# Fancomi2017/InstanceFusion

Hardware: AMD Instinct MI355X
Metric: frames/s + ms/frame (ICP|fuse|instance) at 640x480, 5M surfels, 1/2/4/8 GPU (higher is better)
Workload: dtype f32; 1 GPU; 5000000-surfel map, 640x480 synthetic RGBD stream, 3-level ICP+RGB + surfel fuse + canned-mask instance votes with superpixel refinement; surfels_live=4734799, surfel_slots=4734799, map_order=random, parallelism=replicas x1, loop_frames=90

## Files before the change

include/ifx_c_api.h:

```cpp
#ifndef IFX_C_API_H_
#define IFX_C_API_H_

#include <stdint.h>

#ifdef __cplusplus
extern "C" {
#endif

#define IFX_NUM_INSTANCES 96
#define IFX_VOTE_FLOATS 48

enum {
    IFX_OK = 0,
    IFX_E_INVALID = -1,
    IFX_E_HIP = -2,
    IFX_E_CAPACITY = -3,
    IFX_E_STATE = -4
};

typedef struct ifx_config {
    int32_t width, height;
    float fx, fy, cx, cy;
    int32_t time_delta;
    float confidence;
// ... 46 lines not shown
int ifx_owner_comm_ranks(ifx_t* h);
int ifx_owner_exchange(ifx_t* h, int phase, void** ptrs, int64_t* bytes, int32_t* ops, int max_n);
int ifx_owner_predict_phase(ifx_t* h, int step);
int ifx_owner_of(const float* xyz, int n, int n_ranks, int32_t* out);
int ifx_owner_segmentation_begin(ifx_t* h, const uint8_t* rgb, const uint16_t* depth, const uint8_t* masks, const int32_t* class_ids, int nm, int frame, int flags);
int ifx_owner_segmentation_resume(ifx_t* h);
int ifx_owner_ids_begin(ifx_t* h);
int ifx_owner_ids_resume(ifx_t* h);
int ifx_owner_knn_export(ifx_t* h, void** d_points, void** d_labels, int* n);
int ifx_owner_knn_vote(ifx_t* h, const void* d_all_points, const void* d_all_labels, int n_all, int own_offset);
int ifx_map_seq(ifx_t* h, uint32_t* out, int max_n);
int ifx_map_bounding_boxes(ifx_t* h, int bbox_type, float ratio, float* boxes96x6, float* ground_normal3, float* gc_matrix16, float* inst_matrix96x16,
                           int32_t* ground_votes648);
int ifx_instance_point_cloud(ifx_t* h, int bbox_type, int32_t* counts96, int inst, float* out10, int max_records);
int ifx_view_list_stats(ifx_t* h, int32_t* out4);
int ifx_sync(ifx_t* h);
int ifx_get_pose(ifx_t* h, float* out_pose16);
int ifx_tick(ifx_t* h);
int ifx_trajectory(ifx_t* h, float* out_poses16, int max_frames);
int ifx_tracker_diag(ifx_t* h, float* diag8);
int ifx_tracker_fallbacks(ifx_t* h);
int ifx_tracker_range_exceeded(ifx_t* h);
int ifx_tracker_meet_giveups(ifx_t* h);

int ifx_set_loop_closure(ifx_t* h, int enable, int count_thresh, float err_thresh, float cov_thresh);
int ifx_loop_closure_diag(ifx_t* h, float* out24);
typedef int (*ifx_loop_closure_cb)(ifx_t* h, const float* lc24, void* user);
int ifx_set_loop_closure_callback(ifx_t* h, ifx_loop_closure_cb cb, void* user);
int ifx_sample_graph_model(ifx_t* h, float* out_xyzt, int max_n);
int ifx_loop_closure_constraints(ifx_t* h, float* src3, float* dst3, int32_t* times, int max_n);
int ifx_set_deformation(ifx_t* h, const float* graph16, int n_nodes, int is_fern);
int ifx_adopt_estimated_pose(ifx_t* h);

typedef int (*ifx_fern_cb)(ifx_t* h, void* user);
int ifx_set_fern_callback(ifx_t* h, ifx_fern_cb cb, void* user);
int ifx_adopt_pose(ifx_t* h, const float* pose16);
int ifx_fern_frame(ifx_t* h, uint8_t* img_rgb, float* verts4, float* norms4, uint8_t* inst_rgb);
int ifx_fern_frame_async(ifx_t* h);
int ifx_fern_frame_fetch(ifx_t* h, uint8_t* img_rgb, float* verts4, float* norms4, uint8_t* inst_rgb);
int ifx_track_maps(ifx_t* h, const float* model_v4, const float* model_n4, const uint8_t* model_rgba, const float* cur_v4, const float* cur_n4,
                   const uint8_t* cur_rgba, float* pose16, float* diag8);

typedef struct ifx_soa_view {
    int32_t count;
    int32_t capacity;
    float* d_pos_conf;
// ... 202 lines not shown
```

instancefusion_amd/__init__.py:

```python
from __future__ import annotations

import ctypes as C
import os

import numpy as np

_HERE = os.path.dirname(os.path.abspath(__file__))
LIB_PATH = os.environ.get("IFX_LIB") or os.path.join(_HERE, "libifx.so")
HEADER_PATH = os.path.join(os.path.dirname(_HERE), "include", "ifx_c_api.h")

NUM_INSTANCES = 96
VOTE_FLOATS = 48


class IfxError(RuntimeError):
    pass


class IfxConfig(C.Structure):
    _fields_ = [
        ("width", C.c_int32), ("height", C.c_int32),
        ("fx", C.c_float), ("fy", C.c_float), ("cx", C.c_float), ("cy", C.c_float),
        ("time_delta", C.c_int32), ("confidence", C.c_float), ("depth_cut", C.c_float),
        ("max_depth_processed", C.c_float), ("icp_weight", C.c_float),
# ... 89 lines not shown
    "ifx_owner_process_frame": (C.c_int, [_P, _P, _P, C.c_int64, _P]),
    "ifx_owner_predict": (C.c_int, [_P]),
    "ifx_owner_process_segmentation": (C.c_int, [_P, _P, _P, _P, _P, C.c_int, C.c_int, C.c_int]),
    "ifx_owner_knn_vote_colour": (C.c_int, [_P]),
    "ifx_owner_exchange_stats": (C.c_int, [_P, _P, C.c_int]),
    "ifx_owner_comm_ranks": (C.c_int, [_P]),
    "ifx_map_seq": (C.c_int, [_P, _P, C.c_int]),
    "ifx_prefetch_frame_device": (C.c_int, [_P, _P, _P]),
    "ifx_hint_next_frame_device": (C.c_int, [_P, _P, _P]),
    "ifx_hint_next_frame": (C.c_int, [_P, _P, _P]),
    "ifx_lookahead_stats": (C.c_int, [_P, _P, C.c_int]),
    "ifx_view_list_stats": (C.c_int, [_P, _P]),
    "ifx_map_bounding_boxes": (C.c_int, [_P, C.c_int, C.c_float, _P, _P, _P, _P, _P]),
    "ifx_instance_point_cloud": (C.c_int, [_P, C.c_int, _P, C.c_int, _P, C.c_int]),
    "ifx_sync": (C.c_int, [_P]),
    "ifx_get_pose": (C.c_int, [_P, _P]),
    "ifx_tick": (C.c_int, [_P]),
    "ifx_trajectory": (C.c_int, [_P, _P, C.c_int]),
    "ifx_tracker_diag": (C.c_int, [_P, _P]),
    "ifx_tracker_fallbacks": (C.c_int, [_P]),
    "ifx_build_pyramids": (C.c_int, [_P, _P, _P, _P, _P, _P, _P, C.POINTER(Pyramids)]),
    "ifx_tracker_range_exceeded": (C.c_int, [_P]),
    "ifx_tracker_meet_giveups": (C.c_int, [_P]),
    "ifx_hot_records_stale": (C.c_int, [_P]),
    "ifx_set_loop_closure": (C.c_int, [_P, C.c_int, C.c_int, C.c_float, C.c_float]),
    "ifx_loop_closure_diag": (C.c_int, [_P, _P]),
    "ifx_set_loop_closure_callback": (C.c_int, [_P, _P, _P]),
    "ifx_sample_graph_model": (C.c_int, [_P, _P, C.c_int]),
    "ifx_loop_closure_constraints": (C.c_int, [_P, _P, _P, _P, C.c_int]),
    "ifx_set_deformation": (C.c_int, [_P, _P, C.c_int, C.c_int]),
    "ifx_adopt_estimated_pose": (C.c_int, [_P]),
    "ifx_set_fern_callback": (C.c_int, [_P, _P, _P]),
    "ifx_adopt_pose": (C.c_int, [_P, _P]),
    "ifx_fern_frame": (C.c_int, [_P, _P, _P, _P, _P]),
    "ifx_fern_frame_async": (C.c_int, [_P]),
    "ifx_fern_frame_fetch": (C.c_int, [_P, _P, _P, _P, _P]),
    "ifx_track_maps": (C.c_int, [_P, _P, _P, _P, _P, _P, _P, _P, _P]),
    "ifx_map_view": (C.c_int, [_P, C.POINTER(SoaView)]),
    "ifx_map_count": (C.c_int, [_P]),
    "ifx_map_slots": (C.c_int, [_P]),
    "ifx_map_download": (C.c_int, [_P, C.c_int] + [_P] * 6),
    "ifx_map_upload": (C.c_int, [_P, C.c_int] + [_P] * 6),
    "ifx_set_pose": (C.c_int, [_P, _P, C.c_int]),
    "ifx_compact": (C.c_int, [_P]),
    "ifx_set_option": (C.c_int, [_P, C.c_char_p, C.c_int]),
    "ifx_ids_after": (_P, [_P]),
# ... 238 lines not shown
    @property
    def tick(self):
        return self.L.ifx_tick(self.handle)

    def trajectory(self, max_frames=1 << 16):
        out = np.zeros((max_frames, 16), np.float32)
        n = self._chk(self.L.ifx_trajectory(self.handle, _ptr(out), max_frames), "ifx_trajectory")
        return out[:n].reshape(n, 4, 4).copy()

    def tracker_diag(self):
        out = np.zeros(8, np.float32)
        self._chk(self.L.ifx_tracker_diag(self.handle, _ptr(out)), "ifx_tracker_diag")
        return out

    def tracker_fallbacks(self):
        return self._chk(self.L.ifx_tracker_fallbacks(self.handle), "ifx_tracker_fallbacks")

    def tracker_range_exceeded(self):
        return self._chk(self.L.ifx_tracker_range_exceeded(self.handle), "ifx_tracker_range_exceeded")

    def tracker_meet_giveups(self):
        return self._chk(self.L.ifx_tracker_meet_giveups(self.handle), "ifx_tracker_meet_giveups")

    def set_loop_closure(self, enable=True, count_thresh=35000, err_thresh=5e-5, cov_thresh=1e-5):
        self._chk(self.L.ifx_set_loop_closure(self.handle, int(enable), int(count_thresh), err_thresh, cov_thresh), "ifx_set_loop_closure")

    def loop_closure_diag(self):
        out = np.zeros(24, np.float32)
        self._chk(self.L.ifx_loop_closure_diag(self.handle, _ptr(out)), "ifx_loop_closure_diag")
        return dict(ran=bool(out[0]), inactive_pixels=int(out[1]), icp_error=float(out[2]), icp_count=float(out[3]), cov_ok=bool(out[4]),
                    accepted=bool(out[5]), est_pose=out[6:22].reshape(4, 4).copy(), cov_max=float(out[22]), candidates=int(out[23]))

    def set_loop_closure_callback(self, fn):
        if fn is None:
            self._lc_cb = None
            self._chk(self.L.ifx_set_loop_closure_callback(self.handle, None, None), "ifx_set_loop_closure_callback")
            return

        def tramp(_h, lc, _user):
            try:
                fn(self, np.ctypeslib.as_array(lc, shape=(24,)).copy())
                return 0
            except Exception:
                import traceback

                traceback.print_exc()
# ... 508 lines not shown
```

instancefusion_amd/csrc/ifx_api.hip:

```cpp
#include <climits>
#include "ifx_ctx.h"
#include <string.h>
#include <stdio.h>
#include <algorithm>

int ifx_tracker_external_pose(ifx* h, const float* d_pose16, float weight_mult);
int ifx_tracker_set_weight(ifx* h, float weight_mult);
int ifx_compact_enqueue(ifx* h, int refresh_ids);

void hs_invalidate_view(ifx* h);
static std::string g_err;
extern "C" const char* ifx_global_error(void) { return g_err.c_str(); }
extern "C" const char* ifx_last_error(ifx_t* h) { return h ? h->err.c_str() : g_err.c_str(); }

hipEvent_t ifx_event_get(ifx* h)
{
    if (!h->event_pool.empty()) { hipEvent_t e = h->event_pool.back(); h->event_pool.pop_back(); return e; }
    hipEvent_t e;
    hipEventCreate(&e);
    return e;
}
void ifx_ktime_begin(ifx* h, const char* name, hipEvent_t* a)
{
    (void)name;
// ... 341 lines not shown
    }
    else if (s == "seg_snapshots") { if (value < 1 || value > 8) { h->err = "seg_snapshots must be in [1, 8]"; return IFX_E_INVALID; } h->opt_seg_snapshots = value; }
    else if (s == "ff_rounds") h->opt_ff_rounds = value;
    else if (s == "gn_persist_blocks") { if (value < 1) return IFX_E_INVALID; ifx_drop_tracked(h); h->opt_gn_persist_blocks = value; }
    else if (s == "gn_persist") {
        if (value < 0 || value > 7) { h->err = "gn_persist is a mask of pyramid levels (0..7)"; return IFX_E_INVALID; }
        ifx_drop_tracked(h);
        h->opt_gn_persist = value;
    }
    else if (s == "gn_spin_limit" || s == "gn_fault") {
        if (value < 0) return IFX_E_INVALID;
        ifx_drop_tracked(h);
        HIPCHK(h, hipStreamSynchronize(h->stream));
        HIPCHK(h, hipMemcpy((char*)h->d_state + (s == "gn_fault" ? offsetof(DevState, gn_fault) : offsetof(DevState, gn_spin_limit)), &value, sizeof(int), hipMemcpyHostToDevice));
    }
    else if (s == "gn_prologue") { ifx_drop_tracked(h); h->opt_gn_prologue = value ? 1 : 0; }
    else if (s == "rgb_cand") { ifx_drop_tracked(h); h->opt_rgb_cand = value ? 1 : 0; }
    else if (s == "rgb_fuse") {
        if (value < 0 || value > 7) { h->err = "rgb_fuse is a mask of pyramid levels (0..7)"; return IFX_E_INVALID; }
        ifx_drop_tracked(h);
        h->opt_rgb_fuse = value;
    }
    else if (s == "rgb_fuse_poll") { ifx_drop_tracked(h); h->opt_rgb_fuse_poll = value ? 1 : 0; }
    else if (s == "raster_lds") h->opt_raster_lds = value;
    else if (s == "raster_earlyz") h->opt_raster_earlyz = value;
    else if (s == "pyramid" || s == "fast_odom" || s == "so3" || s == "icp_weight_x1000") {
        if (h->hint_rgb || h->slot[h->tick & 1].for_tick == h->tick) { h->err = "tracker options cannot change while a frame is announced ahead"; return IFX_E_STATE; }
        ifx_drop_tracked(h);
        if (s == "pyramid") h->cfg.pyramid = value ? 1 : 0;
        else if (s == "fast_odom") h->cfg.fast_odom = value ? 1 : 0;
        else if (s == "so3") h->cfg.so3 = value ? 1 : 0;
        else { if (value < 0 || value > 100000) { h->err = "icp_weight_x1000 must be in [0, 100000]"; return IFX_E_INVALID; } h->cfg.icp_weight = value / 1000.f; }
    }
    else { h->err = "unknown option " + s; return IFX_E_INVALID; }
    return IFX_OK;
}

__global__ void k_frame_result(DevState* __restrict__ st, FrameResult* __restrict__ out, float* __restrict__ traj_slot)
{
    if (threadIdx.x < 64) frame_result_wave(st, out, traj_slot, 0, (int)threadIdx.x);
}

static int enqueue_frame_side(ifx* h, int s, int tick, const uint8_t* rgb, const uint16_t* depth, int src_kind)
{
    FrameSlot& f = h->slot[s];
    const int bound = h->cur_slot;
// ... 750 lines not shown
    HIPCHK(h, hipStreamSynchronize(h->stream));
    HIPCHK(h, hipStreamSynchronize(h->stream_b));
    if (h->stream_c) HIPCHK(h, hipStreamSynchronize(h->stream_c));
    ktime_flush(h);
    stage_flush(h);
    if (h->h_result->overflow) { h->err = "surfel store capacity exceeded"; return IFX_E_CAPACITY; }
    return IFX_OK;
}
extern "C" int ifx_tracker_fallbacks(ifx_t* h)
{
    if (!h) return IFX_E_INVALID;
    int r = ifx_sync(h);
    return r ? r : h->h_result->gn_timeout;
}

extern "C" int ifx_hot_records_stale(ifx_t* h)
{
    if (!h) return IFX_E_INVALID;
    HIPCHK(h, hipStreamSynchronize(h->stream));
    int v = 0;
    HIPCHK(h, hipMemcpy(&v, &h->d_state->hot_stale, sizeof(int), hipMemcpyDeviceToHost));
    return v;
}
extern "C" int ifx_tracker_meet_giveups(ifx_t* h)
{
    if (!h) return IFX_E_INVALID;
    int r = ifx_sync(h);
    if (r) return r;
    if (h->stream_c) HIPCHK(h, hipStreamSynchronize(h->stream_c));
    if (h->stream_b) HIPCHK(h, hipStreamSynchronize(h->stream_b));
    long long total = 0;
    for (const DevState* d : {(const DevState*)h->d_state, (const DevState*)h->d_cam_trk}) {
        if (!d) continue;
        int v = 0;
        HIPCHK(h, hipMemcpy(&v, (const char*)d + offsetof(DevState, rgb_meet_giveups), sizeof(int), hipMemcpyDeviceToHost));
        total += v;
    }
    return (int)std::min<long long>(total, 0x7FFFFFFF);
}
extern "C" int ifx_tracker_range_exceeded(ifx_t* h)
{
    if (!h) return IFX_E_INVALID;
    int r = ifx_sync(h);
    if (r) return r;
    if (h->stream_c) HIPCHK(h, hipStreamSynchronize(h->stream_c));
    if (h->stream_b) HIPCHK(h, hipStreamSynchronize(h->stream_b));
    std::vector<const DevState*> sts;
    sts.push_back(h->d_state);
    if (h->d_m2m) sts.push_back(h->d_m2m);
    if (h->d_cam_trk) sts.push_back(h->d_cam_trk);
    for (const FrameSlot& f : h->slot) if (f.so3) sts.push_back(f.so3);
    long long total = 0;
    for (const DevState* d : sts) {
        int v = 0;
        HIPCHK(h, hipMemcpy(&v, (const char*)d + offsetof(DevState, range_exceeded), sizeof(int), hipMemcpyDeviceToHost));
        total += v;
    }
    return (int)std::min<long long>(total, 0x7FFFFFFF);
}

static int frame_sync(ifx* h)
{
// ... 388 lines not shown
```

instancefusion_amd/csrc/ifx_ctx.h:

```cpp
#pragma once
#include <hip/hip_runtime.h>
#include <stdint.h>
#include <string>
#include <vector>
#include <map>
#include "../../include/ifx_c_api.h"
#include "ifx_dev.h"

#ifndef IFX_LIST_SEGS
#define IFX_LIST_SEGS 8
#endif

struct DevState {
    float pose[16];
    float pose_inv[16];
    float last_pose[16];
    float weighting;
    int dense_enough;
    int count;
    int n_dead;
    int n_new;
    int overflow;
    unsigned int r_max_bits;
    float Rprev[9], tprev[3], Rprev_inv[9];
// ... 27 lines not shown
    int vl_valid;
    int vl_scan;
    int vl_age;
    int vl_scans;
    unsigned int vl_n[2];
    unsigned int vl_seg_n[2 * IFX_LIST_SEGS], vl_seg_off[2 * IFX_LIST_SEGS];
    long long dbg[8];
    alignas(64) int gn_res[2];
    unsigned int gn_ticket;
    int gn_pad[13];
    double gn_acc[2 * IFX_ACC_REPL * IFX_ACC_STRIDE];
    double gn_acc2[2 * 2 * IFX_ACC_REPL * IFX_ACC_STRIDE];
    alignas(64) int gn_res2[2 * 16];
    alignas(64) unsigned int gn_bar[4 * 32 * 16];
    int gn_timeout;
    int gn_abort;
    int gn_done_seq;
    int gn_spin_limit, gn_fault;
    alignas(64) double gnp_acc[3 * 2 * IFX_ACC_REPL * IFX_ACC_STRIDE];
    alignas(64) int gnp_res[3 * 16];
    alignas(64) unsigned int gnp_meet[3 * 32];
    alignas(64) double gnp_RRt[2][16];
    int rgb_meet_giveups;
};

struct IdMap { const uint32_t* seq; int own_n; };
__device__ __forceinline__ int idmap_slot(const IdMap& m, int count, int id)
{
    if (m.own_n <= 0) return (id > 0 && id < count) ? id : -1;
    if (id == 0) return -1;
    int lo = 0, hi = count - 1;
    while (lo <= hi) {
        const int mid = (lo + hi) >> 1;
        const unsigned int v = m.seq[mid];
        if (v == (unsigned int)id) return mid;
        if (v < (unsigned int)id) lo = mid + 1; else hi = mid - 1;
    }
    return -1;
}

struct FrameResult {
    float pose[16];
    float diag[8];
    int count, n_dead, n_new, overflow;
    int gn_timeout;
    int seg_counts[2];
// ... 213 lines not shown
    int opt_gn_persist_blocks = 128;
    int opt_gn_persist = 0;
    int gn_max_blocks[4] = {0, 0, 0, 0};
    int opt_rgb_blocks = 0;
    int opt_gn_prologue = 1;
    int oseg_state = 0, oseg_nm = 0, oseg_m = 0, oseg_flags = 0, oseg_pending = 0;
    std::vector<uint8_t> oseg_unavail;
    std::vector<int> oseg_cmp, oseg_bbox, oseg_class;
    hipEvent_t oseg_ev = nullptr;
    int32_t* oseg_rec = nullptr;
    size_t oseg_rec_cap = 0, oseg_rec_bytes = 0;
    int oseg_root = -1, oseg_form = 0, oseg_M = 0, oseg_maxn = 0;
    float oseg_thr = 0.f;
    const char* oseg_who = "";
    void* d_kexp = nullptr;
    int gn_begin_folded = 0;
    int labels_stale_all = 1;
    int opt_raster_lds = 0;
    int opt_view_blocks = 0, opt_clean_blocks = 0, opt_index_blocks = 0;
    int icp_resident_blocks = 1024;
    int opt_res_blocks = 0;
    int opt_rgb_cand = 1;
    int opt_rgb_fuse = 7;
    int opt_rgb_fuse_poll = 1;
    int icp_resident_blocks_fuse = 1024;
    int opt_icp_blocks = 0;
    int opt_raster_tiles = -1;
    int map_external = 0;
    int lc_enable = 0, lc_count_thresh = 35000;
    float lc_err_thresh = 5e-5f, lc_cov_thresh = 1e-5f;
    DevState* d_m2m = nullptr;
    Pyr m2m;
    float *old_vertex = nullptr, *old_normal = nullptr;
    uint8_t *old_image = nullptr, *old_inst = nullptr;
    uint16_t* old_time = nullptr;
    float *act_vertex = nullptr, *act_normal = nullptr;
    uint8_t *act_image = nullptr, *act_inst = nullptr;
    uint16_t* act_time = nullptr;
    size_t lc_half = 0;
    int own_tracked_tick = 0;
    float* h_lc = nullptr;
    int lc_event_valid = 0;
    float* d_graph = nullptr;
    int graph_nodes = 0, graph_is_fern = 0;
    uint8_t* d_inst_gt = nullptr;
    int inst_gt_on = 0;
// ... 208 lines not shown
```

instancefusion_amd/csrc/ifx_track.hip:

```cpp
#include "ifx_ctx.h"
#include "ifx_rgb_chunks.h"
#include <math.h>
#include <string.h>


#define BIL_R 6
#define BIL_BX 32
#define BIL_BY 8
template <bool SHIFTED, bool XCLIP>
__device__ __forceinline__ void bil_window(const uint16_t (*tile)[BIL_BX + 2 * BIL_R + 3], const unsigned char* s_mapx, const unsigned char* s_mapy, int x, int y, int bx, int by, int tx1,
                                           int ty1, unsigned int value, float& sum1, float& sum2)
{
    const float ss = 0.024691358f, sc = 0.000555556f;
    constexpr int D = BIL_R * 2 + 1;
    const float fv = (float)value;
    for (int cy = max(y - D / 2, 0); cy < ty1; ++cy) {
        const int ry = SHIFTED ? (int)s_mapy[cy - by + BIL_R + 1] : cy - by + BIL_R + 1;
        const float dy = (float)y - (float)cy, dy2 = dy * dy;
        float tv[D];
#pragma unroll
        for (int q = 0; q < D; q++) {
            const int col = x - D / 2 + q - bx + BIL_R + 1;
            tv[q] = (float)tile[ry][SHIFTED ? (int)s_mapx[col] : col];
        }
// ... 750 lines not shown
    }
    __shared__ int lds[RED_WAVES][2];
    const int lane = threadIdx.x & 63, wid = threadIdx.x >> 6;
    cnt = wave_sum_i(cnt);
    sig = wave_sum_i(sig);
    if (lane == 0) { lds[wid][0] = cnt; lds[wid][1] = sig; }
    __syncthreads();
    if (threadIdx.x < 2) {
        int s = 0;
        for (int wv = 0; wv < RED_WAVES; wv++) s += lds[wv][threadIdx.x];
        if (!FROM_STATE) partials[bid * 2 + threadIdx.x] = s;
        if (res_total && s) atomicAdd(&res_total[threadIdx.x], s);
    }
}
__global__ __launch_bounds__(RED_THREADS) void k_rgb_residual(const DevState* __restrict__ st, ResArgs ex, float minScale, const int16_t* __restrict__ dIdx,
                                                              const int16_t* __restrict__ dIdy, const float* __restrict__ lastDepth,
                                                              const float* __restrict__ nextDepth, const uint8_t* __restrict__ lastImage,
                                                              const uint8_t* __restrict__ nextImage, Corres8* __restrict__ corres, float maxDepthDelta,
                                                              int w, int h, int* __restrict__ partials)
{
    residual_body(blockIdx.x, gridDim.x, st, ex, minScale, dIdx, dIdy, lastDepth, nextDepth, lastImage, nextImage, corres, maxDepthDelta, w, h, partials);
}

template <bool PRO, bool SC1 = false>
__device__ __forceinline__ int residual_cand_body(int bid, int nblk, const DevState* __restrict__ st, const CandEntry* __restrict__ cand, const unsigned int* __restrict__ cand_n,
                                                   const float* __restrict__ lastDepth, const float* __restrict__ nextDepth, const uint8_t* __restrict__ lastImage,
                                                   const uint8_t* __restrict__ nextImage, Corres8* __restrict__ corres, float maxDepthDelta, int w, int h,
                                                   int* __restrict__ res_total, const GnPro* pro, double* __restrict__ rrt_out)
{
    const int N = w * h;
    const int stride = nblk * RED_THREADS;
    int t = bid * RED_THREADS + threadIdx.x;
    const int n = SC1 ? rgb_chunk_n(cand_n[0], N) : min((int)cand_n[0], N);
    const CandEntry e0 = cand[t < N ? t : 0];
    CandEntry e1 = cand[t + stride < N ? t + stride : 0];
    int pix = t < n ? (int)min(e0.pixel, (uint32_t)(N - 1)) : 0;
    float d1 = nextDepth[pix];
    uint8_t ni = nextImage[pix];
    const float* kk = st->krkinv;
    const float* ktp = st->kt;
    if (PRO) { const float* sp = gn_prologue(st, *pro, rrt_out); kk = sp + 12; ktp = sp + 21; }
    float krk[9];
#pragma unroll
    for (int k = 0; k < 9; k++) krk[k] = kk[k];
    const float kt0 = ktp[0], kt1 = ktp[1], kt2 = ktp[2];
    int cnt = 0, sig = 0;
    while (t < n) {
        const int i = pix / w, j0 = pix - i * w;
        float td1;
        int u0, v0;
        const bool c0 = !(d1 != d1) & rgb_warp(krk, kt0, kt1, kt2, d1, j0, i, w, h, td1, u0, v0);
        const int gj = c0 ? v0 * w + u0 : 0;
        const float d0 = lastDepth[gj];
        const uint8_t li = lastImage[gj];
        const int tn = t + stride, tnn = tn + stride;
        const int pixn = tn < n ? (int)min(e1.pixel, (uint32_t)(N - 1)) : 0;
        const float d1n = nextDepth[pixn];
        const uint8_t nin = nextImage[pixn];
        const CandEntry e2 = cand[tnn < N ? tnn : 0];
        Corres8 c;
        const bool hit = rgb_warp_hit(c0, d0, td1, maxDepthDelta, li != 0);
        const float diff = (float)ni - (float)li;
        c.zx = hit ? (short)u0 : (short)-1; c.zy = hit ? (short)v0 : (short)-1;
        c.diff = hit ? diff : 0.f;
        cnt += hit ? 1 : 0;
        sig += hit ? (int)(diff * diff) : 0;
        if (SC1) {
            unsigned long long bits;
            __builtin_memcpy(&bits, &c, 8);
            __hip_atomic_store(reinterpret_cast<unsigned long long*>(corres + t), bits, __ATOMIC_RELAXED, __HIP_MEMORY_SCOPE_AGENT);
        } else corres[t] = c;
        t = tn; pix = pixn; d1 = d1n; ni = nin; e1 = e2;
    }
    __shared__ int lds[RED_WAVES][2];
    const int lane = threadIdx.x & 63, wid = threadIdx.x >> 6;
    cnt = wave_sum_i(cnt);
    sig = wave_sum_i(sig);
    if (lane == 0) { lds[wid][0] = cnt; lds[wid][1] = sig; }
    __syncthreads();
    if (threadIdx.x < 2) {
        int s = 0;
        for (int wv = 0; wv < RED_WAVES; wv++) s += lds[wv][threadIdx.x];
        if (s) atomicAdd(&res_total[threadIdx.x], s);
    }
    return n;
}

#define RGB_MEET_TICKS 5372u
struct FuseArgs {
    const float* cloud;
    float sobelScale;
    int g;
    unsigned int poll_ticks;
    unsigned int* meet;
    double* clear_acc;
    int* clear_res;
    unsigned int* clear_meet;
    int* range_ctr;
    int* giveups;
};
static_assert(sizeof(Corres8) == 8, "a record is handed over as one 8-byte store");
__device__ __forceinline__ void gnp_clear_set(double* acc, int* res, unsigned int* meet, int* range_ctr)
{
    if (threadIdx.x < 64) {
        const int kind = threadIdx.x >> 5, k = threadIdx.x & 31;
        if (k < 28 && range_exceeded7(kind, k, acc_total(acc + (size_t)kind * IFX_ACC_REPL * IFX_ACC_STRIDE, k))) atomicAdd(range_ctr, 1);
    }
    __syncthreads();
    static_assert(2 * IFX_ACC_REPL * IFX_ACC_STRIDE == RED_THREADS, "one store per thread clears a set's rows");
    __hip_atomic_store(&acc[threadIdx.x], 0.0, __ATOMIC_RELAXED, __HIP_MEMORY_SCOPE_AGENT);
    if (threadIdx.x < 2) __hip_atomic_store(&res[threadIdx.x], 0, __ATOMIC_RELAXED, __HIP_MEMORY_SCOPE_AGENT);
    if (threadIdx.x >= 64 && threadIdx.x < 66) __hip_atomic_store(&meet[(threadIdx.x - 64) * 16], 0u, __ATOMIC_RELAXED, __HIP_MEMORY_SCOPE_AGENT);
}
__device__ __forceinline__ void rgb_fused_step(int bid, int n_wave, Corres8* corres, const CandEntry* __restrict__ cand, int w, int h, float fx, float fy, int* res_total,
                                               double* __restrict__ rgb_acc, const FuseArgs& f)
{
    __shared__ int s_go, s_n;
    __shared__ unsigned int s_chunk;
    asm volatile("s_waitcnt vmcnt(0)" ::: "memory");
    __syncthreads();
    if (threadIdx.x == 0) {
        const unsigned int all = (unsigned int)f.g;
        const unsigned int t = __hip_atomic_fetch_add(&f.meet[0], 1u, __ATOMIC_RELAXED, __HIP_MEMORY_SCOPE_AGENT);
        int go = t + 1u >= all;
        if (!go) {
            if (f.poll_ticks) {
                const unsigned long long t0 = wall_clock64();
                for (;;) {
                    if (__hip_atomic_load(&f.meet[0], __ATOMIC_RELAXED, __HIP_MEMORY_SCOPE_AGENT) >= all) { go = 1; break; }
                    if (wall_clock64() - t0 > (unsigned long long)f.poll_ticks) break;
                    __builtin_amdgcn_s_sleep(2);
                }
            }
            if (!go) atomicAdd(f.giveups, 1);
        }
// ... 27 lines not shown
        }
        __syncthreads();
        if (threadIdx.x == 0) s_chunk = __hip_atomic_fetch_add(&f.meet[16], 1u, __ATOMIC_RELAXED, __HIP_MEMORY_SCOPE_AGENT);
        float X[RGB_CHUNK_IT], Y[RGB_CHUNK_IT], Z[RGB_CHUNK_IT];
#pragma unroll
        for (int u = 0; u < RGB_CHUNK_IT; u++) {
            if (!((c[u].zx >= 0) & (c[u].zx < w) & (c[u].zy >= 0) & (c[u].zy < h))) c[u].zx = -1;
            int g = (c[u].zx >= 0) ? ((int)c[u].zy * w + (int)c[u].zx) * 3 : 0;
            X[u] = f.cloud[g]; Y[u] = f.cloud[g + 1]; Z[u] = f.cloud[g + 2];
        }
#pragma unroll
        for (int u = 0; u < RGB_CHUNK_IT; u++) {
            float row[7] = {0, 0, 0, 0, 0, 0, 0};
            bool found = c[u].zx >= 0;
            if (found) rgb_row(row, sigma, c[u].diff, e[u].gx, e[u].gy, X[u], Y[u], Z[u], fx, fy, f.sobelScale);
            products7<1>(row, found, acc);
        }
        __syncthreads();
        chunk = s_chunk;
    }
    block_sum_exact<29>(acc, rgb_acc, bid % IFX_ACC_REPL);
}

struct PairArgs {
    const float *vmap_curr, *nmap_curr, *vmap_prev, *nmap_prev;
    float fx, fy, cx, cy, distThres, angleThres;
    float minScale, maxDepthDelta;
    const int16_t *dIdx, *dIdy;
    const float *lastDepth, *nextDepth;
    const uint8_t *lastImage, *nextImage;
    Corres8* corres;
    int w, h, nb_icp, nb_res;
    int check_skip;
};
#define IFX_PIN_S(x) asm volatile("" ::"s"(x))
template <bool CHECK_SKIP, bool PRO = false, bool LIST = false, bool FUSE = false>
__global__ __launch_bounds__(RED_THREADS, 4) void k_icp_residual(const DevState* __restrict__ st, int nb_icp, int w, int h, double* __restrict__ gacc, int* __restrict__ gres, PairArgs a, GnPro g,
                                                              double* __restrict__ rrt_store, const CandEntry* __restrict__ cand, const unsigned int* __restrict__ cand_n, FuseArgs f)
{
    static_assert(!FUSE || LIST, "the fused iteration runs over the candidate list");
    if (FUSE) {
        __builtin_assume(st != nullptr);
        if (CHECK_SKIP && st->skip) return;
        const int nb_rgb = (int)gridDim.x - nb_icp;
        if (blockIdx.x == gridDim.x - 1) gnp_clear_set(f.clear_acc, f.clear_res, f.clear_meet, f.range_ctr);
        if ((int)blockIdx.x < nb_rgb) {
            const int n = residual_cand_body<PRO, true>(blockIdx.x, nb_rgb, st, cand, cand_n, a.lastDepth, a.nextDepth, a.lastImage, a.nextImage, a.corres, a.maxDepthDelta, w, h, gres, &g,
                                                        blockIdx.x == 0 ? rrt_store : nullptr);
            rgb_fused_step(blockIdx.x, n, a.corres, cand, w, h, a.fx, a.fy, gres, gacc + IFX_ACC_REPL * IFX_ACC_STRIDE, f);
        } else {
            IcpArgs ia;
            icp_body<false, true, PRO>(blockIdx.x - nb_rgb, nb_icp, st, ia, a.vmap_curr, a.nmap_curr, a.vmap_prev, a.nmap_prev, a.fx, a.fy, a.cx, a.cy, a.distThres, a.angleThres, w, h, gacc, &g,
                                       blockIdx.x == 0 ? rrt_store : nullptr);
        }
        return;
    }
    __builtin_assume(st != nullptr);
    if (CHECK_SKIP && st->skip) return;
    if ((int)blockIdx.x < nb_icp) {
        IcpArgs ia;
        icp_body<false, true, PRO>(blockIdx.x, nb_icp, st, ia, a.vmap_curr, a.nmap_curr, a.vmap_prev, a.nmap_prev, a.fx, a.fy, a.cx, a.cy, a.distThres, a.angleThres, w, h, gacc, &g,
                                   blockIdx.x == 0 ? rrt_store : nullptr);
    } else if (LIST) {
        residual_cand_body<PRO>(blockIdx.x - nb_icp, a.nb_res, st, cand, cand_n, a.lastDepth, a.nextDepth, a.lastImage, a.nextImage, a.corres, a.maxDepthDelta, w, h, gres, &g,
                                blockIdx.x == 0 ? rrt_store : nullptr);
    } else {
        ResArgs ra;
        residual_body<true, PRO>(blockIdx.x - nb_icp, a.nb_res, st, ra, a.minScale, a.dIdx, a.dIdy, a.lastDepth, a.nextDepth, a.lastImage, a.nextImage, a.corres, a.maxDepthDelta, w,
                                 h, nullptr, gres, &g, blockIdx.x == 0 ? rrt_store : nullptr);
// ... 1266 lines not shown
        HIPCHK(h, hipMalloc(&p.vmap_prev[i], n * 12)); HIPCHK(h, hipMalloc(&p.nmap_prev[i], n * 12));
        HIPCHK(h, hipMalloc(&p.last_depth[i], n * 4));
        HIPCHK(h, hipMalloc(&p.last_img[i], n));
        HIPCHK(h, hipMalloc(&p.cloud[i], n * 12));
        HIPCHK(h, hipMalloc(&p.corres[i], n * 8));
    }
    const int maxb = 1024;
    HIPCHK(h, hipMalloc(&p.acc, (3 * IFX_ACC_REPL * IFX_ACC_STRIDE * sizeof(double))));
    HIPCHK(h, hipMemset(p.acc, 0, (3 * IFX_ACC_REPL * IFX_ACC_STRIDE * sizeof(double))));
    {
        int cus = 0, dev = 0;
        hipGetDevice(&dev);
        hipDeviceGetAttribute(&cus, hipDeviceAttributeMultiprocessorCount, dev);
        int occ[4] = {0, 0, 0, 0};
        hipOccupancyMaxActiveBlocksPerMultiprocessor(&occ[0], k_gn_level<1>, RED_THREADS, 0);
        hipOccupancyMaxActiveBlocksPerMultiprocessor(&occ[1], k_gn_level<2>, RED_THREADS, 0);
        hipOccupancyMaxActiveBlocksPerMultiprocessor(&occ[2], k_gn_level<3>, RED_THREADS, 0);
        hipOccupancyMaxActiveBlocksPerMultiprocessor(&occ[3], k_gn_level<4>, RED_THREADS, 0);
        for (int q = 0; q < 4; q++) h->gn_max_blocks[q] = std::max(0, occ[q]) * std::max(0, cus);
        int occ_ir = 0;
        if (hipOccupancyMaxActiveBlocksPerMultiprocessor(&occ_ir, k_icp_residual<false, true>, RED_THREADS, 0) == hipSuccess && occ_ir > 0 && cus > 0) h->icp_resident_blocks = occ_ir * cus;
        int occ_fu = 0;
        if (hipOccupancyMaxActiveBlocksPerMultiprocessor(&occ_fu, k_icp_residual<false, true, true, true>, RED_THREADS, 0) == hipSuccess && occ_fu > 0 && cus > 0) h->icp_resident_blocks_fuse = occ_fu * cus;
    }
    h->res_rows = std::max(maxb, cdiv(h->P, RED_THREADS) + 1);
    HIPCHK(h, hipMalloc(&h->res_partials, (size_t)h->res_rows * 2 * 4));
    HIPCHK(h, hipMalloc(&h->d_out29, 64 * 4));
    HIPCHK(h, hipMalloc(&h->d_ticket, 512));
    HIPCHK(h, hipMemset(h->d_ticket, 0, 512));
    p.res_partials = h->res_partials; p.ticket = h->d_ticket;
    for (int q = 0; q < 2; q++) {
        HIPCHK(h, hipMalloc(&h->slot[q].so3, sizeof(DevState)));
        HIPCHK(h, hipMemset(h->slot[q].so3, 0, sizeof(DevState)));
    }
    ifx_bind_slot(h, 0);
    return IFX_OK;
}

void ifx_bind_slot(ifx* h, int s)
{
    FrameSlot& f = h->slot[s];
    Pyr& p = h->pyr;
    h->cur_slot = s;
    h->rgb = f.rgb; h->depth_raw = f.depth_raw; h->depth_filt = f.depth_filt; h->dm = f.dm; h->dmf = f.dmf;
    for (int i = 0; i < IFX_NUM_PYRS; i++) {
        p.depth_tmp[i] = (i == 0) ? f.depth_filt : f.depth_tmp[i]; p.vmap_curr[i] = f.vmap_curr[i]; p.nmap_curr[i] = f.nmap_curr[i];
// ... 122 lines not shown
    int blocks = 0;
    for (int i = 0; i < IFX_NUM_PYRS; i++) {
        float div = (float)(1 << i);
        float fx = h->cfg.fx / div, fy = h->cfg.fy / div;
        FrameLevel& L = fl.l[i];
        L.depth = p.depth_tmp[i]; L.img = p.next_img[i]; L.vmap = p.vmap_curr[i]; L.nmap = p.nmap_curr[i]; L.dx = p.didx[i]; L.dy = p.didy[i];
        L.w = p.w[i]; L.h = p.h[i]; L.tiles_x = cdiv(p.w[i], 32); L.first_block = blocks;
        L.fx_inv = 1.f / fx; L.fy_inv = 1.f / fy; L.cx = h->cfg.cx / div; L.cy = h->cfg.cy / div;
        L.cand = p.cand[i]; L.cand_n = p.cand_n[i]; L.minScale = rgb_min_scale(i);
        blocks += L.tiles_x * cdiv(p.h[i], 8);
    }
    fl.cutoff = h->cfg.max_depth_processed;
    LAUNCH(h, "frame_maps", dim3(blocks), dim3(256), k_frame_maps, fl);
}

int ifx_comm_ready(ifx* h);
int ifx_comm_allreduce_f64(ifx* h, double* d_ptr, int n);
static_assert(IFX_NUM_PYRS == 3, "level names");
static inline const char* icp_name_rows(int level) { static const char* const n[3] = {"icp_residual_rows@L0", "icp_residual_rows@L1", "icp_residual_rows@L2"}; return n[level]; }
static inline const char* icp_name(int level) { static const char* const n[3] = {"icp_residual@L0", "icp_residual@L1", "icp_residual@L2"}; return n[level]; }
static inline const char* rgb_name(int level) { static const char* const n[3] = {"rgb_step_solve@L0", "rgb_step_solve@L1", "rgb_step_solve@L2"}; return n[level]; }

using IcpResidualKernel = decltype(&k_icp_residual<false>);
static IcpResidualKernel icp_residual_kernel(bool check_skip, bool pro, bool list, bool fuse)
{
    static const IcpResidualKernel k[2][2][3] = {
        {{k_icp_residual<false, false>, k_icp_residual<false, false, true>, k_icp_residual<false, false, true, true>},
         {k_icp_residual<false, true>, k_icp_residual<false, true, true>, k_icp_residual<false, true, true, true>}},
        {{k_icp_residual<true, false>, k_icp_residual<true, false, true>, k_icp_residual<true, false, true, true>},
         {k_icp_residual<true, true>, k_icp_residual<true, true, true>, k_icp_residual<true, true, true, true>}}};
    return k[check_skip][pro][fuse ? 2 : list ? 1 : 0];
}
using RgbStepSolveKernel = decltype(&k_rgb_step_solve<false>);
static RgbStepSolveKernel rgb_step_solve_kernel(bool check_skip, bool list)
{
    static const RgbStepSolveKernel k[2][2] = {{k_rgb_step_solve<false>, k_rgb_step_solve<false, true>}, {k_rgb_step_solve<true>, k_rgb_step_solve<true, true>}};
    return k[check_skip][list];
}

struct RunPlan {
    int icp, rgb;
    int iterations[IFX_NUM_PYRS], first;
    bool finer[IFX_NUM_PYRS];
    float next_div[IFX_NUM_PYRS];
    int persist_q[IFX_NUM_PYRS], persist_nb[IFX_NUM_PYRS];
    bool cand_run;
    bool pro;
    int n_pro;
};
static RunPlan plan_run(ifx* h, const Pyr& p, float icp_weight, bool frame_tracker)
{
    const ifx_config& c = h->cfg;
    RunPlan pl;
    const int icp = icp_weight > 0, rgb = icp_weight < 100;
// ... 172 lines not shown
static void emit_iteration(TrackRun& r, int i, int j, const LevelLaunch& L)
{
    ifx* const h = r.h;
    DevState* const st = r.st;
    const RunPlan& pl = r.plan;
    const PairArgs& pa = L.pa;
    const int tail_k = r.tail_k++;
    GnPro gp;
    gp.k = tail_k; gp.icp = pl.icp; gp.rgb = pl.rgb; gp.icp_weight = r.icp_weight; gp.nfx = pa.fx; gp.nfy = pa.fy; gp.ncx = pa.cx; gp.ncy = pa.cy; gp.ki = kinv_of(pa.fx, pa.fy, pa.cx, pa.cy);
    const bool it_pro = pl.pro && tail_k < pl.n_pro;
    const bool fuse = pl.cand_run && it_pro && tail_k < pl.n_pro - 1 && (h->opt_rgb_fuse & (1 << i));
    double* const ga = it_pro ? gnp_acc_of(st, tail_k % 3) : gn_acc_of(st);
    int* const gr = it_pro ? gnp_res_of(st, tail_k % 3) : gn_res_of(st);
    double* const rrt_store = gnp_rrt_of(st, (tail_k + 1) & 1);
    FuseArgs fa;
    memset(&fa, 0, sizeof(fa));
    PairArgs paf = pa;
    if (fuse) {
        paf.nb_res = std::max(1, std::min(rgb_fuse_blocks(h, pa.w * pa.h), h->icp_resident_blocks_fuse - pa.nb_icp));
        const int cs = (tail_k + 1) % 3;
        fa.cloud = r.p.cloud[i]; fa.sobelScale = (float)GN_SOBEL_SCALE; fa.g = paf.nb_res; fa.poll_ticks = h->opt_rgb_fuse_poll ? RGB_MEET_TICKS : 0u;
        fa.meet = gnp_meet_of(st, tail_k % 3); fa.clear_acc = gnp_acc_of(st, cs); fa.clear_res = gnp_res_of(st, cs); fa.clear_meet = gnp_meet_of(st, cs);
        fa.range_ctr = (int*)((char*)st + offsetof(DevState, range_exceeded)); fa.giveups = (int*)((char*)st + offsetof(DevState, rgb_meet_giveups));
    }
    LAUNCH(h, icp_name(i), dim3(paf.nb_icp + paf.nb_res), dim3(RED_THREADS), icp_residual_kernel(!r.frame_tracker, it_pro && tail_k > 0, pl.cand_run, fuse), st, paf.nb_icp, paf.w, paf.h, ga, gr, paf,
           gp, rrt_store, L.cl, L.cln, fa);
    if (fuse) return;
    StepArgs sa2 = step_args(r, i, j);
    sa2.nb = L.nb_rgb; sa2.nb_icp = L.nb; sa2.nb_res = L.nbr; sa2.check_skip = r.frame_tracker ? 0 : 1; sa2.lctr = r.frame_tracker ? h->d_list_ctr : (unsigned int*)nullptr;
    sa2.pro = it_pro ? (tail_k == pl.n_pro - 1 ? 2 : 1) : 0; sa2.pro_k = tail_k;
    r.ended = r.ended || sa2.end_run;
    LAUNCH(h, rgb_name(i), dim3(L.nb_rgb), dim3(RED_THREADS), rgb_step_solve_kernel(!r.frame_tracker, pl.cand_run), st, sa2.nb, sa2.rgb, sa2.w, sa2.h, sa2, L.cl, L.cln);
}

static void tracker_run(ifx* h, DevState* st, Pyr& p, float icp_weight, int so3, float weight_mult, int commit, bool frame_tracker, int keep_last = 0)
{
    const ifx_config& c = h->cfg;
    TrackRun r = {h, st, p, icp_weight, weight_mult, commit, frame_tracker, plan_run(h, p, icp_weight, frame_tracker), 0, 0, false};
    const RunPlan& pl = r.plan;
    if (frame_tracker && h->gn_begin_folded) h->gn_begin_folded = 0;
    else {
        const float div = (float)(1 << (pl.first < 0 ? 0 : pl.first));
        LAUNCH(h, "track_gn_begin", dim3(1), dim3(64), k_track_gn_begin, st, h->slot[h->cur_slot].so3, so3, c.fx / div, c.fy / div, c.cx / div, c.cy / div, keep_last, h->opt_gn_persist ? 1 : 0);
    }
    if (frame_tracker && h->own && h->opt_own_track_rows && ifx_comm_ready(h) && h->own_track_rank < 0) emit_rows_run(r);
    else
        for (int i = IFX_NUM_PYRS - 1; i >= 0; i--) {
            if (i == 0 && frame_tracker) ifx_enqueue_hinted_frame_side(h);
// ... 554 lines not shown
```

Baseline: 1851 frames/s.

## Let fused RGB blocks process their own records and adopt orphaned blocks' shares

Adds an 'own-records' variant of the fused ICP/RGB iteration. Each RGB block keeps its first correspondence in registers and, after the meet barrier, sums only its strided share of the candidate records. The last-arriving block adopts the shares of blocks that gave up waiting, tracked through orphan and taken bitmasks. The aim is to replace the single-block or serialized RGB reduction after the meet with distributed per-block work. In exchange the kernel gets more complex cross-block synchronization, and its occupancy may cap the resident fused block count.

```diff
diff --git a/include/ifx_c_api.h b/include/ifx_c_api.h
--- a/include/ifx_c_api.h
+++ b/include/ifx_c_api.h
@@ -92,6 +92,7 @@
 int ifx_tracker_fallbacks(ifx_t* h);
 int ifx_tracker_range_exceeded(ifx_t* h);
 int ifx_tracker_meet_giveups(ifx_t* h);
+int ifx_tracker_meet_adopted(ifx_t* h);
 
 int ifx_set_loop_closure(ifx_t* h, int enable, int count_thresh, float err_thresh, float cov_thresh);
 int ifx_loop_closure_diag(ifx_t* h, float* out24);
diff --git a/instancefusion_amd/__init__.py b/instancefusion_amd/__init__.py
--- a/instancefusion_amd/__init__.py
+++ b/instancefusion_amd/__init__.py
@@ -135,6 +135,7 @@
     "ifx_build_pyramids": (C.c_int, [_P, _P, _P, _P, _P, _P, _P, C.POINTER(Pyramids)]),
     "ifx_tracker_range_exceeded": (C.c_int, [_P]),
     "ifx_tracker_meet_giveups": (C.c_int, [_P]),
+    "ifx_tracker_meet_adopted": (C.c_int, [_P]),
     "ifx_hot_records_stale": (C.c_int, [_P]),
     "ifx_set_loop_closure": (C.c_int, [_P, C.c_int, C.c_int, C.c_float, C.c_float]),
     "ifx_loop_closure_diag": (C.c_int, [_P, _P]),
@@ -419,6 +420,9 @@
     def tracker_meet_giveups(self):
         return self._chk(self.L.ifx_tracker_meet_giveups(self.handle), "ifx_tracker_meet_giveups")
 
+    def tracker_meet_adopted(self):
+        return self._chk(self.L.ifx_tracker_meet_adopted(self.handle), "ifx_tracker_meet_adopted")
+
     def set_loop_closure(self, enable=True, count_thresh=35000, err_thresh=5e-5, cov_thresh=1e-5):
         self._chk(self.L.ifx_set_loop_closure(self.handle, int(enable), int(count_thresh), err_thresh, cov_thresh), "ifx_set_loop_closure")
 
diff --git a/instancefusion_amd/csrc/ifx_api.hip b/instancefusion_amd/csrc/ifx_api.hip
--- a/instancefusion_amd/csrc/ifx_api.hip
+++ b/instancefusion_amd/csrc/ifx_api.hip
@@ -387,6 +387,11 @@
         h->opt_rgb_fuse = value;
     }
     else if (s == "rgb_fuse_poll") { ifx_drop_tracked(h); h->opt_rgb_fuse_poll = value ? 1 : 0; }
+    else if (s == "rgb_own") {
+        if (value < 0 || value > 7) { h->err = "rgb_own is a mask of pyramid levels (0..7)"; return IFX_E_INVALID; }
+        ifx_drop_tracked(h);
+        h->opt_rgb_own = value;
+    }
     else if (s == "raster_lds") h->opt_raster_lds = value;
     else if (s == "raster_earlyz") h->opt_raster_earlyz = value;
     else if (s == "pyramid" || s == "fast_odom" || s == "so3" || s == "icp_weight_x1000") {
@@ -1183,7 +1188,7 @@
     HIPCHK(h, hipMemcpy(&v, &h->d_state->hot_stale, sizeof(int), hipMemcpyDeviceToHost));
     return v;
 }
-extern "C" int ifx_tracker_meet_giveups(ifx_t* h)
+static int ifx_tracker_meet_counter(ifx_t* h, size_t offset)
 {
     if (!h) return IFX_E_INVALID;
     int r = ifx_sync(h);
@@ -1194,11 +1199,13 @@
     for (const DevState* d : {(const DevState*)h->d_state, (const DevState*)h->d_cam_trk}) {
         if (!d) continue;
         int v = 0;
-        HIPCHK(h, hipMemcpy(&v, (const char*)d + offsetof(DevState, rgb_meet_giveups), sizeof(int), hipMemcpyDeviceToHost));
+        HIPCHK(h, hipMemcpy(&v, (const char*)d + offset, sizeof(int), hipMemcpyDeviceToHost));
         total += v;
     }
     return (int)std::min<long long>(total, 0x7FFFFFFF);
 }
+extern "C" int ifx_tracker_meet_giveups(ifx_t* h) { return ifx_tracker_meet_counter(h, offsetof(DevState, rgb_meet_giveups)); }
+extern "C" int ifx_tracker_meet_adopted(ifx_t* h) { return ifx_tracker_meet_counter(h, offsetof(DevState, rgb_meet_adopted)); }
 extern "C" int ifx_tracker_range_exceeded(ifx_t* h)
 {
     if (!h) return IFX_E_INVALID;
diff --git a/instancefusion_amd/csrc/ifx_ctx.h b/instancefusion_amd/csrc/ifx_ctx.h
--- a/instancefusion_amd/csrc/ifx_ctx.h
+++ b/instancefusion_amd/csrc/ifx_ctx.h
@@ -73,6 +73,7 @@
     alignas(64) unsigned int gnp_meet[3 * 32];
     alignas(64) double gnp_RRt[2][16];
     int rgb_meet_giveups;
+    int rgb_meet_adopted;
 };
 
 struct IdMap { const uint32_t* seq; int own_n; };
@@ -332,6 +333,7 @@
     int opt_res_blocks = 0;
     int opt_rgb_cand = 1;
     int opt_rgb_fuse = 7;
+    int opt_rgb_own = 7;
     int opt_rgb_fuse_poll = 1;
     int icp_resident_blocks_fuse = 1024;
     int opt_icp_blocks = 0;
diff --git a/instancefusion_amd/csrc/ifx_rgb_own.h b/instancefusion_amd/csrc/ifx_rgb_own.h
--- /dev/null
+++ b/instancefusion_amd/csrc/ifx_rgb_own.h
@@ -0,0 +1,15 @@
+#pragma once
+
+#include "ifx_rgb_chunks.h"
+
+#define RGB_OWN_MAX_G 64
+#define RGB_OWN_IT 2
+
+IFX_HD inline int rgb_own_first(int b, int tid) { return b * RGB_CHUNK_THREADS + tid; }
+IFX_HD inline int rgb_own_rounds(int n, int g, int first)
+{
+    if (g <= 0 || first < 0 || first >= n) return 0;
+    return (n - 1 - first) / (g * RGB_CHUNK_THREADS) + 1;
+}
+IFX_HD inline int rgb_own_record(int g, int first, int k) { return first + k * (g * RGB_CHUNK_THREADS); }
+IFX_HD inline int rgb_own_block_rounds(int n, int g, int b) { return rgb_own_rounds(n, g, rgb_own_first(b, 0)); }
diff --git a/instancefusion_amd/csrc/ifx_track.hip b/instancefusion_amd/csrc/ifx_track.hip
--- a/instancefusion_amd/csrc/ifx_track.hip
+++ b/instancefusion_amd/csrc/ifx_track.hip
@@ -1,5 +1,6 @@
 #include "ifx_ctx.h"
 #include "ifx_rgb_chunks.h"
+#include "ifx_rgb_own.h"
 #include <math.h>
 #include <string.h>
 
@@ -796,12 +797,15 @@
     residual_body(blockIdx.x, gridDim.x, st, ex, minScale, dIdx, dIdy, lastDepth, nextDepth, lastImage, nextImage, corres, maxDepthDelta, w, h, partials);
 }
 
-template <bool PRO, bool SC1 = false>
+struct RgbOwn { Corres8 c; int16_t gx, gy; float X, Y, Z; };
+template <bool PRO, bool SC1 = false, bool OWN = false>
 __device__ __forceinline__ int residual_cand_body(int bid, int nblk, const DevState* __restrict__ st, const CandEntry* __restrict__ cand, const unsigned int* __restrict__ cand_n,
                                                    const float* __restrict__ lastDepth, const float* __restrict__ nextDepth, const uint8_t* __restrict__ lastImage,
                                                    const uint8_t* __restrict__ nextImage, Corres8* __restrict__ corres, float maxDepthDelta, int w, int h,
-                                                   int* __restrict__ res_total, const GnPro* pro, double* __restrict__ rrt_out)
-{
+                                                   int* __restrict__ res_total, const GnPro* pro, double* __restrict__ rrt_out, const float* __restrict__ cloud = nullptr,
+                                                   RgbOwn* own = nullptr)
+{
+    static_assert(!OWN || SC1, "the own-records form is a form of the fused iteration");
     const int N = w * h;
     const int stride = nblk * RED_THREADS;
     int t = bid * RED_THREADS + threadIdx.x;
@@ -819,6 +823,8 @@
     for (int k = 0; k < 9; k++) krk[k] = kk[k];
     const float kt0 = ktp[0], kt1 = ktp[1], kt2 = ktp[2];
     int cnt = 0, sig = 0;
+    bool first = OWN;
+    if (OWN) { own->c.zx = -1; own->c.zy = -1; own->c.diff = 0.f; own->gx = e0.gx; own->gy = e0.gy; own->X = own->Y = own->Z = 0.f; }
     while (t < n) {
         const int i = pix / w, j0 = pix - i * w;
         float td1;
@@ -844,6 +850,12 @@
             __builtin_memcpy(&bits, &c, 8);
             __hip_atomic_store(reinterpret_cast<unsigned long long*>(corres + t), bits, __ATOMIC_RELAXED, __HIP_MEMORY_SCOPE_AGENT);
         } else corres[t] = c;
+        if (OWN && first) {
+            first = false;
+            own->c = c;
+            const int g = hit ? gj * 3 : 0;
+            own->X = cloud[g]; own->Y = cloud[g + 1]; own->Z = cloud[g + 2];
+        }
         t = tn; pix = pixn; d1 = d1n; ni = nin; e1 = e2;
     }
     __shared__ int lds[RED_WAVES][2];
@@ -872,7 +884,11 @@
     unsigned int* clear_meet;
     int* range_ctr;
     int* giveups;
+    int* adopted;
 };
+#define RGB_MEET_ORPHAN 18
+#define RGB_MEET_TAKEN 20
+static_assert(RGB_MEET_ORPHAN % 2 == 0 && RGB_MEET_TAKEN == RGB_MEET_ORPHAN + 2 && RGB_MEET_ORPHAN > 16 && RGB_MEET_TAKEN + 2 <= 32, "two aligned 64-bit words in the set's second line");
 static_assert(sizeof(Corres8) == 8, "a record is handed over as one 8-byte store");
 __device__ __forceinline__ void gnp_clear_set(double* acc, int* res, unsigned int* meet, int* range_ctr)
 {
@@ -885,6 +901,8 @@
     __hip_atomic_store(&acc[threadIdx.x], 0.0, __ATOMIC_RELAXED, __HIP_MEMORY_SCOPE_AGENT);
     if (threadIdx.x < 2) __hip_atomic_store(&res[threadIdx.x], 0, __ATOMIC_RELAXED, __HIP_MEMORY_SCOPE_AGENT);
     if (threadIdx.x >= 64 && threadIdx.x < 66) __hip_atomic_store(&meet[(threadIdx.x - 64) * 16], 0u, __ATOMIC_RELAXED, __HIP_MEMORY_SCOPE_AGENT);
+    if (threadIdx.x >= 128 && threadIdx.x < 130)
+        __hip_atomic_store(reinterpret_cast<unsigned long long*>(meet + RGB_MEET_ORPHAN) + (threadIdx.x - 128), 0ull, __ATOMIC_RELAXED, __HIP_MEMORY_SCOPE_AGENT);
 }
 __device__ __forceinline__ void rgb_fused_step(int bid, int n_wave, Corres8* corres, const CandEntry* __restrict__ cand, int w, int h, float fx, float fy, int* res_total,
                                                double* __restrict__ rgb_acc, const FuseArgs& f)
@@ -958,6 +976,113 @@
     block_sum_exact<29>(acc, rgb_acc, bid % IFX_ACC_REPL);
 }
 
+__device__ __forceinline__ void rgb_own_step(int bid, int n_wave, const RgbOwn& own, Corres8* corres, const CandEntry* __restrict__ cand, int w, int h, float fx, float fy, int* res_total,
+                                             double* __restrict__ rgb_acc, const FuseArgs& f)
+{
+    __shared__ int s_go, s_n;
+    __shared__ unsigned int s_adopt[2];
+    unsigned long long* const orphan = reinterpret_cast<unsigned long long*>(f.meet + RGB_MEET_ORPHAN);
+    unsigned long long* const taken = reinterpret_cast<unsigned long long*>(f.meet + RGB_MEET_TAKEN);
+    asm volatile("s_waitcnt vmcnt(0)" ::: "memory");
+    __syncthreads();
+    if (threadIdx.x == 0) {
+        const unsigned int all = (unsigned int)f.g;
+        const unsigned long long bit = 1ull << (bid & 63);
+        const unsigned int t = __hip_atomic_fetch_add(&f.meet[0], 1u, __ATOMIC_RELAXED, __HIP_MEMORY_SCOPE_AGENT);
+        int go = t + 1u >= all ? 2 : 0;
+        if (!go) {
+            if (f.poll_ticks) {
+                const unsigned long long t0 = wall_clock64();
+                for (;;) {
+                    if (__hip_atomic_load(&f.meet[0], __ATOMIC_RELAXED, __HIP_MEMORY_SCOPE_AGENT) >= all) { go = 1; break; }
+                    if (wall_clock64() - t0 > (unsigned long long)f.poll_ticks) break;
+                    __builtin_amdgcn_s_sleep(2);
+                }
+            }
+            if (!go) {
+                const unsigned long long before = __hip_atomic_fetch_or(orphan, bit, __ATOMIC_RELAXED, __HIP_MEMORY_SCOPE_AGENT);
+                asm volatile("s_waitcnt vmcnt(0)" ::"v"(before) : "memory");
+                if (__hip_atomic_load(&f.meet[0], __ATOMIC_RELAXED, __HIP_MEMORY_SCOPE_AGENT) >= all)
+                    go = (__hip_atomic_fetch_or(taken, bit, __ATOMIC_RELAXED, __HIP_MEMORY_SCOPE_AGENT) & bit) ? 0 : 1;
+                if (!go) atomicAdd(f.giveups, 1);
+            }
+        }
+        s_go = go;
+        s_n = n_wave;
+    }
+    __syncthreads();
+    const int go = __builtin_amdgcn_readfirstlane(s_go);
+    if (!go) return;
+    const bool last = go == 2;
+    const int n = __builtin_amdgcn_readfirstlane(s_n);
+    const int g = f.g;
+    if (!last && rgb_own_block_rounds(n, g, bid) == 0) return;
+    const int r_cnt = __hip_atomic_load(&res_total[0], __ATOMIC_RELAXED, __HIP_MEMORY_SCOPE_AGENT), r_sig = __hip_atomic_load(&res_total[1], __ATOMIC_RELAXED, __HIP_MEMORY_SCOPE_AGENT);
+    unsigned long long orph = 0;
+    if (last && threadIdx.x == 0) orph = __hip_atomic_load(orphan, __ATOMIC_RELAXED, __HIP_MEMORY_SCOPE_AGENT);
+    const float sigma = rgb_sigma(r_cnt, r_sig);
+    double acc[29];
+#pragma unroll
+    for (int k = 0; k < 29; k++) acc[k] = 0.0;
+    auto in_image = [&](const Corres8& c) { return (c.zx >= 0) & (c.zx < w) & (c.zy >= 0) & (c.zy < h); };
+    {
+        float row[7] = {0, 0, 0, 0, 0, 0, 0};
+        const bool found = in_image(own.c);
+        if (found) rgb_row(row, sigma, own.c.diff, own.gx, own.gy, own.X, own.Y, own.Z, fx, fy, f.sobelScale);
+        products7<1>(row, found, acc);
+    }
+    auto step_share = [&](int b, int k0) {
+        const int first = rgb_own_first(b, (int)threadIdx.x);
+        const int rounds = rgb_own_rounds(n, g, first);
+        for (int k = k0; k < rounds; k += RGB_OWN_IT) {
+            Corres8 c[RGB_OWN_IT];
+            CandEntry e[RGB_OWN_IT];
+#pragma unroll
+            for (int u = 0; u < RGB_OWN_IT; u++) {
+                const bool in = k + u < rounds;
+                const int kk = rgb_own_record(g, first, in ? k + u : k);
+                const unsigned long long bits = __hip_atomic_load(reinterpret_cast<unsigned long long*>(corres + kk), __ATOMIC_RELAXED, __HIP_MEMORY_SCOPE_AGENT);
+                __builtin_memcpy(&c[u], &bits, 8);
+                e[u] = cand[kk];
+                if (!in) c[u].zx = -1;
+            }
+            float X[RGB_OWN_IT], Y[RGB_OWN_IT], Z[RGB_OWN_IT];
+#pragma unroll
+            for (int u = 0; u < RGB_OWN_IT; u++) {
+                if (!in_image(c[u])) c[u].zx = -1;
+                const int gi = (c[u].zx >= 0) ? ((int)c[u].zy * w + (int)c[u].zx) * 3 : 0;
+                X[u] = f.cloud[gi]; Y[u] = f.cloud[gi + 1]; Z[u] = f.cloud[gi + 2];
+            }
+#pragma unroll
+            for (int u = 0; u < RGB_OWN_IT; u++) {
+                float row[7] = {0, 0, 0, 0, 0, 0, 0};
+                const bool found = c[u].zx >= 0;
+                if (found) rgb_row(row, sigma, c[u].diff, e[u].gx, e[u].gy, X[u], Y[u], Z[u], fx, fy, f.sobelScale);
+                products7<1>(row, found, acc);
+            }
+        }
+    };
+    step_share(bid, 1);
+    if (last) {
+        if (threadIdx.x == 0) {
+            unsigned long long mine = 0;
+            if (orph) {
+                mine = orph & ~__hip_atomic_fetch_or(taken, orph, __ATOMIC_RELAXED, __HIP_MEMORY_SCOPE_AGENT);
+                if (mine) atomicAdd(f.adopted, __popcll(mine));
+            }
+            s_adopt[0] = (unsigned int)mine; s_adopt[1] = (unsigned int)(mine >> 32);
+        }
+        __syncthreads();
+        unsigned long long mine = (unsigned long long)__builtin_amdgcn_readfirstlane(s_adopt[0]) | ((unsigned long long)__builtin_amdgcn_readfirstlane(s_adopt[1]) << 32);
+        while (mine) {
+            const int o = __ffsll((long long)mine) - 1;
+            mine &= mine - 1;
+            if (o < g) step_share(o, 0);
+        }
+    }
+    block_sum_exact<29>(acc, rgb_acc, bid % IFX_ACC_REPL);
+}
+
 struct PairArgs {
     const float *vmap_curr, *nmap_curr, *vmap_prev, *nmap_prev;
     float fx, fy, cx, cy, distThres, angleThres;
@@ -970,17 +1095,23 @@
     int check_skip;
 };
 #define IFX_PIN_S(x) asm volatile("" ::"s"(x))
-template <bool CHECK_SKIP, bool PRO = false, bool LIST = false, bool FUSE = false>
+template <bool CHECK_SKIP, bool PRO = false, bool LIST = false, bool FUSE = false, bool OWN = false>
 __global__ __launch_bounds__(RED_THREADS, 4) void k_icp_residual(const DevState* __restrict__ st, int nb_icp, int w, int h, double* __restrict__ gacc, int* __restrict__ gres, PairArgs a, GnPro g,
                                                               double* __restrict__ rrt_store, const CandEntry* __restrict__ cand, const unsigned int* __restrict__ cand_n, FuseArgs f)
 {
     static_assert(!FUSE || LIST, "the fused iteration runs over the candidate list");
+    static_assert(!OWN || FUSE, "the own-records form is a form of the fused iteration");
     if (FUSE) {
         __builtin_assume(st != nullptr);
         if (CHECK_SKIP && st->skip) return;
         const int nb_rgb = (int)gridDim.x - nb_icp;
         if (blockIdx.x == gridDim.x - 1) gnp_clear_set(f.clear_acc, f.clear_res, f.clear_meet, f.range_ctr);
-        if ((int)blockIdx.x < nb_rgb) {
+        if (OWN && (int)blockIdx.x < nb_rgb) {
+            RgbOwn own;
+            const int n = residual_cand_body<PRO, true, true>(blockIdx.x, nb_rgb, st, cand, cand_n, a.lastDepth, a.nextDepth, a.lastImage, a.nextImage, a.corres, a.maxDepthDelta, w, h, gres, &g,
+                                                              blockIdx.x == 0 ? rrt_store : nullptr, f.cloud, &own);
+            rgb_own_step(blockIdx.x, n, own, a.corres, cand, w, h, a.fx, a.fy, gres, gacc + IFX_ACC_REPL * IFX_ACC_STRIDE, f);
+        } else if ((int)blockIdx.x < nb_rgb) {
             const int n = residual_cand_body<PRO, true>(blockIdx.x, nb_rgb, st, cand, cand_n, a.lastDepth, a.nextDepth, a.lastImage, a.nextImage, a.corres, a.maxDepthDelta, w, h, gres, &g,
                                                         blockIdx.x == 0 ? rrt_store : nullptr);
             rgb_fused_step(blockIdx.x, n, a.corres, cand, w, h, a.fx, a.fy, gres, gacc + IFX_ACC_REPL * IFX_ACC_STRIDE, f);
@@ -2293,6 +2424,9 @@
         if (hipOccupancyMaxActiveBlocksPerMultiprocessor(&occ_ir, k_icp_residual<false, true>, RED_THREADS, 0) == hipSuccess && occ_ir > 0 && cus > 0) h->icp_resident_blocks = occ_ir * cus;
         int occ_fu = 0;
         if (hipOccupancyMaxActiveBlocksPerMultiprocessor(&occ_fu, k_icp_residual<false, true, true, true>, RED_THREADS, 0) == hipSuccess && occ_fu > 0 && cus > 0) h->icp_resident_blocks_fuse = occ_fu * cus;
+        int occ_own = 0;
+        if (hipOccupancyMaxActiveBlocksPerMultiprocessor(&occ_own, k_icp_residual<false, true, true, true, true>, RED_THREADS, 0) == hipSuccess && occ_own > 0 && cus > 0)
+            h->icp_resident_blocks_fuse = std::min(h->icp_resident_blocks_fuse, occ_own * cus);
     }
     h->res_rows = std::max(maxb, cdiv(h->P, RED_THREADS) + 1);
     HIPCHK(h, hipMalloc(&h->res_partials, (size_t)h->res_rows * 2 * 4));
@@ -2461,14 +2595,14 @@
 static inline const char* rgb_name(int level) { static const char* const n[3] = {"rgb_step_solve@L0", "rgb_step_solve@L1", "rgb_step_solve@L2"}; return n[level]; }
 
 using IcpResidualKernel = decltype(&k_icp_residual<false>);
-static IcpResidualKernel icp_residual_kernel(bool check_skip, bool pro, bool list, bool fuse)
-{
-    static const IcpResidualKernel k[2][2][3] = {
-        {{k_icp_residual<false, false>, k_icp_residual<false, false, true>, k_icp_residual<false, false, true, true>},
-         {k_icp_residual<false, true>, k_icp_residual<false, true, true>, k_icp_residual<false, true, true, true>}},
-        {{k_icp_residual<true, false>, k_icp_residual<true, false, true>, k_icp_residual<true, false, true, true>},
-         {k_icp_residual<true, true>, k_icp_residual<true, true, true>, k_icp_residual<true, true, true, true>}}};
-    return k[check_skip][pro][fuse ? 2 : list ? 1 : 0];
+static IcpResidualKernel icp_residual_kernel(bool check_skip, bool pro, bool list, bool fuse, bool own)
+{
+    static const IcpResidualKernel k[2][2][4] = {
+        {{k_icp_residual<false, false>, k_icp_residual<false, false, true>, k_icp_residual<false, false, true, true>, k_icp_residual<false, false, true, true, true>},
+         {k_icp_residual<false, true>, k_icp_residual<false, true, true>, k_icp_residual<false, true, true, true>, k_icp_residual<false, true, true, true, true>}},
+        {{k_icp_residual<true, false>, k_icp_residual<true, false, true>, k_icp_residual<true, false, true, true>, k_icp_residual<true, false, true, true, true>},
+         {k_icp_residual<true, true>, k_icp_residual<true, true, true>, k_icp_residual<true, true, true, true>, k_icp_residual<true, true, true, true, true>}}};
+    return k[check_skip][pro][fuse ? (own ? 3 : 2) : list ? 1 : 0];
 }
 using RgbStepSolveKernel = decltype(&k_rgb_step_solve<false>);
 static RgbStepSolveKernel rgb_step_solve_kernel(bool check_skip, bool list)
@@ -2687,8 +2821,10 @@
         fa.cloud = r.p.cloud[i]; fa.sobelScale = (float)GN_SOBEL_SCALE; fa.g = paf.nb_res; fa.poll_ticks = h->opt_rgb_fuse_poll ? RGB_MEET_TICKS : 0u;
         fa.meet = gnp_meet_of(st, tail_k % 3); fa.clear_acc = gnp_acc_of(st, cs); fa.clear_res = gnp_res_of(st, cs); fa.clear_meet = gnp_meet_of(st, cs);
         fa.range_ctr = (int*)((char*)st + offsetof(DevState, range_exceeded)); fa.giveups = (int*)((char*)st + offsetof(DevState, rgb_meet_giveups));
-    }
-    LAUNCH(h, icp_name(i), dim3(paf.nb_icp + paf.nb_res), dim3(RED_THREADS), icp_residual_kernel(!r.frame_tracker, it_pro && tail_k > 0, pl.cand_run, fuse), st, paf.nb_icp, paf.w, paf.h, ga, gr, paf,
+        fa.adopted = (int*)((char*)st + offsetof(DevState, rgb_meet_adopted));
+    }
+    const bool own = fuse && (h->opt_rgb_own & (1 << i)) && paf.nb_res <= RGB_OWN_MAX_G;
+    LAUNCH(h, icp_name(i), dim3(paf.nb_icp + paf.nb_res), dim3(RED_THREADS), icp_residual_kernel(!r.frame_tracker, it_pro && tail_k > 0, pl.cand_run, fuse, own), st, paf.nb_icp, paf.w, paf.h, ga, gr, paf,
            gp, rrt_store, L.cl, L.cln, fa);
     if (fuse) return;
     StepArgs sa2 = step_args(r, i, j);
```

After: 1898 frames/s (median of 6 runs). 1.03x the previous value.
